# LouisPwr/CarpeDeam

Measured on AMD Instinct MI355X. Metric: corrected bases/sec on 50M×100bp synthetic reads (dhigh), 1/2/4/8 GPU, higher is better.
Workload: dtype u8 (2-bit packed bases; int32 scores; software x87 f80 likelihood sums)

## Files before the change

### carpedeam_amd/csrc/extend.hip

```cpp
#include "scan.h"

#include <cmath>
#include <cstring>

#include "seqdb.h"
#include "devutil.h"

namespace {

struct Cand {
    int qs, qe, ds, de;
    uint32_t target, alnLen, dbLen, qLen;
    float seqId, rySeqId;
    double sLenNorm;
    uint32_t pieceStart, pieceLen;
    uint32_t tKey;
};

struct ExtArgs {
    MetaWoff woff; MetaLen len; MetaHasN hasN; MetaExt ext; MetaKey key; MetaRaw hasRaw;
    const uint32_t *codes, *nmask; const uint8_t *raw;
    const uint64_t *aoff;
    const AlnRec *rec;
    const uint32_t *active; const unsigned int *nActive;
// ... 77 lines not shown
        long long start;
        if (c.ds == 0 && (uint32_t) c.qe == qLen - 1) start = (long long) qLen + c.qs;
        else if (c.qs == 0 && (uint32_t) c.de == tLen - 1) start = (long long) qLen - (long long) (c.dbLen - c.alnLen);
        else continue;
        if ((long long) x < start || (long long) x >= start + (long long) c.dbLen) continue;
        uint32_t tc; bool tn;
        targetBaseAt(A, c.target, (uint32_t) ((long long) x - start), tc, tn);
        cnt[tn ? 0u : fwdBase(tc)]++;
    }
    code = 0; isN = true;
    if (cnt[0] + cnt[1] + cnt[2] + cnt[3] < A.minCov) return;
    uint32_t mx = 0; int nMax = 0;
    for (uint32_t j = 0; j < 4; j++) {
        if (cnt[j] > mx) { mx = cnt[j]; code = j; nMax = 1; } else if (cnt[j] == mx && mx > 0) nMax++;
    }
    isN = nMax != 1;
    if (isN) code = 0;
}


__device__ __forceinline__ bool rightStarts(int ds, int qe, uint32_t qLen) { return (uint32_t) ds == 0 && (uint32_t) qe == (qLen - 1); }
__device__ __forceinline__ bool leftStarts(int qs, int de, uint32_t dbLen) { return (uint32_t) qs == 0 && (uint32_t) de == (dbLen - 1); }

struct Overlap { bool left, right; uint32_t q0, t0, ncol; };
__device__ __forceinline__ Overlap endOverlap(const Cand &c, uint32_t qLen) {
    Overlap o;
    o.right = rightStarts(c.ds, c.qe, qLen); o.left = leftStarts(c.qs, c.de, c.dbLen);
    const uint32_t offset = c.dbLen - c.alnLen;
    if (o.left) { o.t0 = offset; o.q0 = 0; o.ncol = min(c.dbLen - offset, qLen); }
    else { o.t0 = 0; o.q0 = qLen - c.alnLen; o.ncol = min(c.alnLen, c.dbLen); }
    return o;
}
__device__ __forceinline__ void noteOverlap(const Overlap &o, uint32_t tot, uint32_t &maxLeft, uint32_t &maxRight) {
    if (o.left && tot > maxLeft) maxLeft = tot; else if (o.right && tot > maxRight) maxRight = tot;
}
__device__ __forceinline__ void plainOverlapMax(const Cand &c, uint32_t qLen, uint32_t &maxLeft, uint32_t &maxRight) {
    const Overlap o = endOverlap(c, qLen);
    noteOverlap(o, o.ncol, maxLeft, maxRight);
}

__device__ __forceinline__ uint32_t damageClass(uint32_t ti, uint32_t dbLen) { return ti < 5 ? ti : (ti >= dbLen - 5 ? 6 + (ti - (dbLen - 5)) : 5); }

__device__ __forceinline__ void countMatchesWordsAt(const uint32_t *__restrict__ codes, uint32_t qw, uint32_t qLast, uint32_t q0, uint32_t tw, uint32_t tLast, uint32_t t0, uint32_t n, int &idCnt, int &idRy) {
    uint32_t mm = 0, ry = 0;
    for (uint32_t k = 0; k < n; k += 16) {
        const uint32_t x = cdm_window16(codes, qw, q0 + k, qLast) ^ cdm_window16(codes, tw, t0 + k, tLast);
        uint32_t any = (x | (x >> 1)) & 0x55555555u, lowbit = x & 0x55555555u;
        const uint32_t rem = n - k;
        if (rem < 16) { const uint32_t m = (1u << (2 * rem)) - 1u; any &= m; lowbit &= m; }
        mm += __popc(any); ry += __popc(lowbit);
    }
    idCnt = (int) (n - mm); idRy = (int) (n - ry);
}
__device__ __forceinline__ void countMatchesLetters(const ExtArgs &A, uint32_t q, uint32_t qw, uint32_t q0, uint32_t t, uint32_t tw, uint32_t t0, uint32_t n, int &idCnt, int &idRy) {
    idCnt = 0; idRy = 0;
    for (uint32_t i = 0; i < n; i++) {
        uint32_t qc, tc; bool qn, tn;
        letterOf(A, q, qw, q0 + i, qc, qn); letterOf(A, t, tw, t0 + i, tc, tn);
        idCnt += ((qn ? 4u : qc) == (tn ? 4u : tc));
        idRy += (ryClass(qn ? 0u : qc) == ryClass(tn ? 0u : tc));
    }
}

template <typename F>
__device__ __forceinline__ void walkPlainColumns(const ExtArgs &A, const VQuery &Q, const Cand &c, const Overlap &o, F f) {
    const uint32_t qw = Q.qw, tw = A.woff[c.target];
    const uint32_t qLast = (Q.qLen0 + 15) / 16 - 1, tLast = (c.dbLen + 15) / 16 - 1;
    uint32_t qNext = cdm_window16(A.codes, qw, o.q0, qLast), tNext = cdm_window16(A.codes, tw, o.t0, tLast);
    for (uint32_t k = 0; k < o.ncol; k += 16) {
        uint32_t qwin = qNext, twin = tNext;
        if (k + 16 < o.ncol) { qNext = cdm_window16(A.codes, qw, o.q0 + k + 16, qLast); tNext = cdm_window16(A.codes, tw, o.t0 + k + 16, tLast); }
        const uint32_t m = min(16u, o.ncol - k);
        for (uint32_t j = 0; j < m; j++) {
            f(damageClass(o.t0 + k + j, c.dbLen), qwin & 3u, twin & 3u);
            qwin >>= 2; twin >>= 2;
        }
    }
}

__device__ void updateIds(const ExtArgs &A, const VQuery &Q, Cand &c, uint32_t &maxLeft, uint32_t &maxRight, const ConsList *cons = nullptr) {
    const uint32_t qLen = Q.total;
    const Overlap o = endOverlap(c, qLen);
    int idCnt = 0, idRy = 0; uint32_t tot = 0;
    if (cons && (o.left || o.right)) {
        if (c.dbLen - c.alnLen > qLen) A.flags[0] = 1u;
        else {
            const uint32_t c0 = qLen + o.q0 - o.t0;
            for (uint32_t j = 0; j < c.dbLen && c0 + j < 3 * qLen; j++) {
                uint32_t qc, tc; bool qn, tn;
                consensusAt(A, Q, *cons, c0 + j, qc, qn); targetBaseAt(A, c.target, j, tc, tn);
                if (qn || tn) continue;
                idCnt += (qc == tc); idRy += (ryClass(qc) == ryClass(tc)); tot++;
            }
        }
    } else
    if (o.left || o.right) {
        if (Q.plain && !A.hasN[c.target]) {
            countMatchesWordsAt(A.codes, Q.qw, (Q.qLen0 + 15) / 16 - 1, o.q0, A.woff[c.target], (c.dbLen + 15) / 16 - 1, o.t0, o.ncol, idCnt, idRy);
            tot = o.ncol;
        } else
        for (uint32_t i = 0; i < o.ncol; i++) {
            uint32_t qc, tc; bool qn, tn;
            Q.baseAt(o.q0 + i, qc, qn); targetBaseAt(A, c.target, o.t0 + i, tc, tn);
            if (qn || tn) continue;
            idCnt += (qc == tc); idRy += (ryClass(qc) == ryClass(tc)); tot++;
        }
// ... 5 lines not shown
__device__ bool scoreCand(const ExtArgs &A, const VQuery &Q, Cand &c, uint32_t maxLeft, uint32_t maxRight, const double *logLik ,
                          const ConsList *cons = nullptr, const X87 *logLikX = nullptr ) {
    const uint32_t qLen = Q.total;
    const Overlap o = endOverlap(c, qLen);
    const uint32_t maxAln = o.left ? maxLeft : maxRight;
    X87 lik = x87_zero();
    uint32_t alnCount = 0;
    if (cons && (o.left || o.right)) {
        if (c.dbLen - c.alnLen > qLen) A.flags[0] = 1u;
        else {
            const uint32_t c0 = qLen + o.q0 - o.t0;
            uint32_t tIdx = 0;
            for (uint32_t j = 0; j < c.dbLen && c0 + j < 3 * qLen; j++) {
                uint32_t qc, tc; bool qn, tn;
                targetBaseAt(A, c.target, j, tc, tn);
                if (!tn) tIdx++;
                if (tn) continue;
                consensusAt(A, Q, *cons, c0 + j, qc, qn);
                if (qn) continue;
                alnCount++;
                lik = x87_add(lik, x87_from_double(logLik[(damageClass(tIdx - 1, c.dbLen) * 4 + fwdBase(qc)) * 4 + fwdBase(tc)]));
            }
        }
    } else
    if (o.left || o.right) {
        if (Q.plain && !A.hasN[c.target]) {
            if (logLikX) walkPlainColumns(A, Q, c, o, [&](uint32_t cls, uint32_t qb, uint32_t tb) { lik = x87_acc(lik, logLikX[(cls * 4 + qb) * 4 + tb]); });
            else walkPlainColumns(A, Q, c, o, [&](uint32_t cls, uint32_t qb, uint32_t tb) { lik = x87_acc(lik, x87_from_double(logLik[(cls * 4 + qb) * 4 + tb])); });
            alnCount = o.ncol;
        } else {
            uint32_t tIdx = 0;
            if (o.left) for (uint32_t j = 0; j < o.t0; j++) { uint32_t tc; bool tn; targetBaseAt(A, c.target, j, tc, tn); tIdx += !tn; }
            for (uint32_t i = 0; i < o.ncol; i++) {
                uint32_t qc, tc; bool qn, tn;
                Q.baseAt(o.q0 + i, qc, qn); targetBaseAt(A, c.target, o.t0 + i, tc, tn);
                if (!tn) tIdx++;
                if (qn || tn) continue;
                alnCount++;
                lik = x87_add(lik, x87_from_double(logLik[(damageClass(tIdx - 1, c.dbLen) * 4 + fwdBase(qc)) * 4 + fwdBase(tc)]));
            }
        }
    }
    const uint32_t excess = maxAln - alnCount;
    const float pen = (float) excess * A.excessLog;
    lik = x87_add(lik, x87_from_double((double) pen));
    const double randAln = (double) ((float) maxAln * A.randLog);
    c.sLenNorm = x87_to_double(lik);
    X87 neg = lik; neg.s ^= 1u;
    const double x = x87_to_double(x87_add(x87_from_double(randAln), neg));
    if (A.ratioWindow > 0.0 && fabs(x - A.ratioLogit) <= A.ratioWindow) A.flags[2] = 1u;
    return x < A.ratioLogit;
}

__device__ int scoreCandApprox(const ExtArgs &A, const VQuery &Q, const Cand &c, uint32_t maxLeft, uint32_t maxRight, const double *logLik, double &sLenNorm, float &bound) {
    const Overlap o = endOverlap(c, Q.total);
    const uint32_t maxAln = o.left ? maxLeft : maxRight;
    double sum = 0.0, mag = 0.0;
    walkPlainColumns(A, Q, c, o, [&](uint32_t cls, uint32_t qb, uint32_t tb) {
        const double t = logLik[(cls * 4 + qb) * 4 + tb];
        sum = __dadd_rn(sum, t); mag = __dadd_rn(mag, fabs(t));
    });
    const uint32_t excess = maxAln - o.ncol;
    const double pen = (double) ((float) excess * A.excessLog);
    sum = __dadd_rn(sum, pen); mag = __dadd_rn(mag, fabs(pen));
    const double randAln = (double) ((float) maxAln * A.randLog);
    const double b = fmax((double) (o.ncol + 8u) * 0x1p-52 * (mag + fabs(randAln)) * (double) A.marginScale, A.ratioWindow);
    sLenNorm = sum; bound = (float) b * 1.0000002f + 1e-37f;
    const double x = __dadd_rn(randAln, -sum);
    if (x < A.ratioLogit - b) return 1;
    if (x > A.ratioLogit + b) return 0;
    return -1;
}

struct CandTest { bool ok, left, right; uint32_t alnLen; float seqId, rySeqId; };
__device__ __forceinline__ uint32_t recAlnLen(const AlnRec &rec) { return (uint32_t) max(abs(rec.qEnd - rec.qStart), abs(rec.dbEnd - rec.dbStart)) + 1u; }
__device__ __forceinline__ CandTest candidateTest(const ExtArgs &A, const AlnRec &rec, uint32_t q, const SeqMeta &qm, const SeqMeta &tm) {
    CandTest T; T.ok = false; T.alnLen = 0; T.seqId = rec.seqId; T.rySeqId = 0.f;
    T.right = rightStarts(rec.dbStart, rec.qEnd, qm.len); T.left = leftStarts(rec.qStart, rec.dbEnd, tm.len);
    if (!T.right && !T.left) return T;
    if (rec.qStart > rec.qEnd) return T;
    T.alnLen = recAlnLen(rec);
    if (rec.target != qm.key) {
        int idCnt, idRy;
        const uint32_t n = (uint32_t) (rec.qEnd - rec.qStart + 1);
        if (((qm.flags | tm.flags) & 1u) == 0) countMatchesWordsAt(A.codes, qm.woff, (qm.len + 15) / 16 - 1, (uint32_t) rec.qStart, tm.woff, (tm.len + 15) / 16 - 1, (uint32_t) rec.dbStart, n, idCnt, idRy);
        else countMatchesLetters(A, q, qm.woff, (uint32_t) rec.qStart, rec.target, tm.woff, (uint32_t) rec.dbStart, n, idCnt, idRy);
        T.seqId = static_cast<float>(idCnt) / T.alnLen; T.rySeqId = static_cast<float>(idRy) / T.alnLen;
    }
    const bool wasExtended = (tm.flags >> 1) & 1u, noOffset = (tm.len - T.alnLen) == 0;
    T.ok = !wasExtended && T.alnLen >= 30 && T.seqId >= A.seqIdThr && !noOffset;
    return T;
}
__device__ __forceinline__ void candFill(Cand &c, const AlnRec &rec, uint32_t alnLen, const SeqMeta &tm, uint32_t qLen0, float seqId, float rySeqId, uint32_t r) {
    const uint32_t tLen = tm.len; c.tKey = tm.key;
    c.qs = rec.qStart; c.qe = rec.qEnd; c.ds = rec.dbStart; c.de = rec.dbEnd; c.target = rec.target; c.alnLen = alnLen; c.dbLen = tLen;
    c.qLen = qLen0; c.seqId = seqId; c.rySeqId = rySeqId; c.sLenNorm = 0; c.pieceStart = r; c.pieceLen = 0;
}

__device__ __forceinline__ bool scoredAtAll(const ExtArgs &A, const Cand &c, uint32_t qKey) {
    const bool notInside = c.dbLen != c.alnLen, rightStart = c.ds == 0, leftStart = c.qs == 0, notId = c.tKey != qKey;
    return (rightStart || leftStart) && notInside && notId && c.rySeqId >= A.rySeqIdThr && c.seqId >= A.seqIdThr;
}

struct QLists { uint32_t *heap, *park, *left, *right; };
__device__ __forceinline__ QLists queryLists(const ExtArgs &A, uint64_t r0, uint32_t nRec) {
    QLists L; L.heap = A.lists + 4 * r0; L.park = L.heap + nRec; L.left = L.park + nRec; L.right = L.left + nRec;
    return L;
}
__device__ __forceinline__ void queryView(VQuery &Q, const ExtArgs &A, uint32_t q, const SeqMeta &qm, const Cand *cand = nullptr, const QLists *L = nullptr, bool grown = false) {
    Q.a = &A; Q.q = q; Q.qLen0 = qm.len; Q.qw = qm.woff; Q.cand = cand; Q.leftL = L ? L->left : nullptr; Q.rightL = L ? L->right : nullptr;
    Q.nL = grown ? A.nLeft[q] : 0; Q.nR = grown ? A.nRight[q] : 0; Q.leftTotal = grown ? A.leftTotal[q] : 0;
    Q.total = grown ? A.newLen[q] : qm.len; Q.plain = !grown && (qm.flags & 1u) == 0;
}

__device__ __forceinline__ void loadLogLik(const ExtArgs &A, double *sLogLik, X87 *sLogLikX = nullptr) {
    for (int i = threadIdx.x; i < 11 * 16; i += blockDim.x) {
        const double v = (&A.lut->logLik[0][0][0][0])[i];
        sLogLik[i] = v;
        if (sLogLikX) sLogLikX[i] = x87_from_double(v);
    }
}

struct Heap {
    uint32_t *h; uint32_t n; const Cand *cand;
    __device__ bool less(uint32_t x, uint32_t y) const { return cand[x].sLenNorm < cand[y].sLenNorm; }
    __device__ void siftUp(uint32_t hole, uint32_t top, uint32_t value) {
        while (hole > top) { const uint32_t parent = (hole - 1) / 2; if (!less(h[parent], value)) break; h[hole] = h[parent]; hole = parent; }
        h[hole] = value;
    }
    __device__ void push(uint32_t v) { n++; siftUp(n - 1, 0, v); }
    __device__ uint32_t pop() {
        const uint32_t topV = h[0];
        const uint32_t len = n - 1;
        if (len > 0) {
            const uint32_t value = h[len];
            uint32_t hole = 0, child = 0;
            while (child < (len - 1) / 2) { child = 2 * (child + 1); if (less(h[child], h[child - 1])) child--; h[hole] = h[child]; hole = child; }
            if ((len & 1u) == 0 && child == (len - 2) / 2) { child = 2 * (child + 1); h[hole] = h[child - 1]; hole = child - 1; }
// ... 108 lines not shown
    const unsigned int item = blockIdx.x * blockDim.x + threadIdx.x;
    if (item >= *A.nActive) return;
    const uint32_t q = A.active[item];
    const uint64_t r0 = A.aoff[q], r1 = A.aoff[q + 1];
    const uint32_t nRec = (uint32_t) (r1 - r0);
    const SeqMeta *meta = A.len.m;
    const SeqMeta qm = meta[q];
    const uint32_t qLen0 = qm.len, qKey = qm.key;
    Cand *cand = A.cand + r0;
    const QLists L = queryLists(A, r0, nRec);
    VQuery Q; queryView(Q, A, q, qm, cand, &L);

    uint32_t nCand = 0;
    AlnRec recN = A.rec[r0]; SeqMeta tmN = meta[recN.target];
    for (uint32_t r = 0; r < nRec; r++) {
        const AlnRec rec = recN; const SeqMeta tm = tmN;
        if (r + 1 < nRec) { recN = A.rec[r0 + r + 1]; tmN = meta[recN.target]; }
        if (A.scores) A.scores[r0 + r] = NAN;
        const CandTest T = candidateTest(A, rec, q, qm, tm);
        if (T.ok) candFill(cand[nCand++], rec, T.alnLen, tm, qLen0, T.seqId, T.rySeqId, r);
    }
    if (nCand == 0) { A.newLen[q] = 0; return; }
    uint32_t maxLeft = 0, maxRight = 0;
    ConsList consAll; consAll.cand = cand; consAll.idx = nullptr; consAll.n = nCand; consAll.qKey = qKey;
    const ConsList *cons0 = A.unsafe ? &consAll : nullptr;
    for (uint32_t k = 0; k < nCand; k++) {
        Cand &c = cand[k];
        if (A.unsafe) updateIds(A, Q, c, maxLeft, maxRight, cons0);
        else if (Q.plain && !A.hasN[c.target] && c.target != qKey) plainOverlapMax(c, qLen0, maxLeft, maxRight);
        else updateIds(A, Q, c, maxLeft, maxRight);
    }
    Heap heap; heap.h = L.heap; heap.n = 0; heap.cand = cand;
    for (uint32_t k = 0; k < nCand; k++) {
        Cand &c = cand[k];
        if (scoredAtAll(A, c, qKey)) {
            const bool pass = scoreCand(A, Q, c, maxLeft, maxRight, sLogLik, cons0);
            if (A.scores) A.scores[r0 + c.pieceStart] = c.sLenNorm;
            if (pass) heap.push(k);
        }
    }
    extendLoop(A, Q, cand, heap, L, maxLeft, maxRight, sLogLik, qKey, q);
}

constexpr int XR_NT = 512, XR_T = 448, XR_QCAP = 512, XR_LCAP = 1024, XR_BINS = 32;
struct XrArgs {
    const uint32_t *winQ;
    float2 *lite;
    double *sLen;
    float *sBound;
    uint32_t *qMax;
    uint32_t *elig;
    uint32_t *pushBits;
    uint32_t *work; unsigned int *nWork, *fallback;
};
__global__ void k_xr_windows(const uint64_t *__restrict__ aoff, uint32_t n, uint32_t nWin, uint32_t *__restrict__ winQ) {
    const uint32_t b = blockIdx.x * blockDim.x + threadIdx.x;
    if (b > nWin) return;
    const uint64_t x = (uint64_t) b * XR_T;
    uint32_t lo = 0, hi = n;
    while (lo < hi) { const uint32_t mid = lo + (hi - lo) / 2; if (aoff[mid] < x) lo = mid + 1; else hi = mid; }
    winQ[b] = lo;
}
#ifndef CDM_XRS_MINB
#define CDM_XRS_MINB 3
#endif
__global__ __launch_bounds__(XR_NT, CDM_XRS_MINB) void k_xr_score(ExtArgs A, XrArgs X) {
    A.raw = nullptr;
    __shared__ double sLogLik[11 * 16];
    __shared__ X87 sLogLikX[11 * 16];
    __shared__ uint32_t sOff[XR_QCAP + 1], sMaxL[XR_QCAP], sMaxR[XR_QCAP], sCnt[XR_QCAP];
    __shared__ uint32_t sListA[XR_LCAP], sListB[XR_LCAP];
    __shared__ uint8_t sBinOf[XR_LCAP];
    __shared__ unsigned int sElig, sBinCnt[XR_BINS], sBinBase[XR_BINS];
    loadLogLik(A, sLogLik, sLogLikX);
    const uint32_t qFirst = X.winQ[blockIdx.x], qEnd = X.winQ[blockIdx.x + 1];
    const SeqMeta *meta = A.len.m;
    for (uint32_t qb = qFirst; qb < qEnd; qb += XR_QCAP) {
        const uint32_t nq = min((uint32_t) XR_QCAP, qEnd - qb);
        __syncthreads();
        const uint64_t ra = A.aoff[qb];
        for (uint32_t i = threadIdx.x; i <= nq; i += XR_NT) sOff[i] = (uint32_t) (A.aoff[qb + i] - ra);
        for (uint32_t i = threadIdx.x; i < nq; i += XR_NT) { sMaxL[i] = 0; sMaxR[i] = 0; sCnt[i] = 0; }
        if (threadIdx.x == 0) sElig = 0;
        if (threadIdx.x < XR_BINS) sBinCnt[threadIdx.x] = 0;
        __syncthreads();
        const uint32_t nr = sOff[nq];
        for (uint32_t base = 0; base < nr; base += XR_NT) {
            const uint32_t i = base + threadIdx.x;
            if (i >= nr) continue;
            uint32_t lo = 0, hi = nq;
            while (hi - lo > 1) { const uint32_t mid = (lo + hi) / 2; if (sOff[mid] <= i) lo = mid; else hi = mid; }
            const uint32_t ord = lo, q = qb + ord;
            float2 out = make_float2(NAN, 0.f);
            if (sOff[ord + 1] - sOff[ord] > 1) {
                const AlnRec rec = A.rec[ra + i]; const SeqMeta qm = meta[q];
                const bool rightStart = rightStarts(rec.dbStart, rec.qEnd, qm.len);
                const bool maybe = !(rec.qStart > rec.qEnd) && (rightStart || rec.qStart == 0);
                if (maybe) {
                    const SeqMeta tm = meta[rec.target];
                    const CandTest T = candidateTest(A, rec, q, qm, tm);
                    if (T.ok) {
                        Cand c; candFill(c, rec, T.alnLen, tm, qm.len, T.seqId, T.rySeqId, i);
                        if (T.left && T.right) X.fallback[0] = 1u;
                        uint32_t mL = 0, mR = 0;
                        if (((qm.flags | tm.flags) & 1u) == 0 && rec.target != qm.key) plainOverlapMax(c, qm.len, mL, mR);
                        else { VQuery Q; queryView(Q, A, q, qm); updateIds(A, Q, c, mL, mR); }
                        if (mL) atomicMax(&sMaxL[ord], mL);
                        if (mR) atomicMax(&sMaxR[ord], mR);
                        out = make_float2(c.seqId, c.rySeqId);
                        if (scoredAtAll(A, c, qm.key)) {
                            const uint32_t slot = atomicAdd(&sElig, 1u);
                            if (slot < XR_LCAP) {
                                const uint32_t bin = min((uint32_t) XR_BINS - 1u, T.alnLen >> 3);
                                sListA[slot] = i; sBinOf[slot] = (uint8_t) bin; atomicAdd(&sBinCnt[bin], 1u);
                            } else X.elig[ra + slot] = i;
                        }
                    }
                }
            }
            if (out.x == out.x) X.lite[ra + i] = out;
            if (A.scores && sOff[ord + 1] - sOff[ord] > 1) A.scores[ra + i] = NAN;
        }
        __syncthreads();
        const uint32_t nElig = sElig, nListed = min(nElig, (uint32_t) XR_LCAP);
        if (threadIdx.x == 0) { unsigned int acc = 0; for (int b = 0; b < XR_BINS; b++) { sBinBase[b] = acc; acc += sBinCnt[b]; } }
        __syncthreads();
        for (uint32_t k = threadIdx.x; k < nListed; k += XR_NT) sListB[atomicAdd(&sBinBase[sBinOf[k]], 1u)] = sListA[k];
        __syncthreads();
        for (uint32_t k = threadIdx.x; k < nElig; k += XR_NT) {
            const uint32_t i = k < XR_LCAP ? sListB[k] : X.elig[ra + k];
            uint32_t lo = 0, hi = nq;
            while (hi - lo > 1) { const uint32_t mid = (lo + hi) / 2; if (sOff[mid] <= i) lo = mid; else hi = mid; }
            const uint32_t ord = lo, q = qb + ord;
            const float2 l = X.lite[ra + i];
            const AlnRec rec = A.rec[ra + i]; const SeqMeta tm = meta[rec.target], qm = meta[q];
            Cand c; candFill(c, rec, recAlnLen(rec), tm, qm.len, l.x, l.y, i);
            VQuery Q; queryView(Q, A, q, qm);
            bool pass; float bnd = 0.f;
            int quick = -1;
            if (!A.scores && Q.plain && (tm.flags & 1u) == 0) { double sl; quick = scoreCandApprox(A, Q, c, sMaxL[ord], sMaxR[ord], sLogLik, sl, bnd); c.sLenNorm = sl; }
            if (quick < 0) { pass = scoreCand(A, Q, c, sMaxL[ord], sMaxR[ord], sLogLik, nullptr, sLogLikX); bnd = 0.f; }
            else pass = quick != 0;
            if (A.scores) A.scores[ra + i] = c.sLenNorm;
            if (pass) {
                X.sLen[ra + i] = c.sLenNorm; X.sBound[ra + i] = bnd;
                atomicAdd(&sCnt[ord], 1u);
                atomicOr(&X.pushBits[(ra + i) >> 5], 1u << ((ra + i) & 31u));
            }
        }
        __syncthreads();
        for (uint32_t i0 = 0; i0 < nq; i0 += XR_NT) {
            const uint32_t i = i0 + threadIdx.x;
            const bool has = i < nq && sCnt[i] != 0;
            const uint32_t slot = cdm_block_append(X.nWork, has);
            if (has) { X.work[slot] = qb + i; X.qMax[2 * (size_t) (qb + i)] = sMaxL[i]; X.qMax[2 * (size_t) (qb + i) + 1] = sMaxR[i]; }
        }
    }
}

#ifndef CDM_XRE_MINW
#define CDM_XRE_MINW 8
#endif
__global__ __launch_bounds__(64, CDM_XRE_MINW) void k_xr_extend(ExtArgs A, XrArgs X) {
    A.raw = nullptr;
    __shared__ double sLogLik[11 * 16];
    loadLogLik(A, sLogLik);
    __syncthreads();
    const unsigned int item = blockIdx.x * blockDim.x + threadIdx.x;
    if (item >= *X.nWork) return;
    const uint32_t q = X.work[item];
    const SeqMeta *meta = A.len.m;
    const SeqMeta qm = meta[q];
    const uint64_t r0 = A.aoff[q];
    const uint32_t nRec = (uint32_t) (A.aoff[q + 1] - r0);
    Cand *cand = A.cand + r0;
    const QLists L = queryLists(A, r0, nRec);
    VQuery Q; queryView(Q, A, q, qm, cand, &L);
    Heap heap; heap.h = L.heap; heap.n = 0; heap.cand = cand;
    uint32_t nCand = 0;
    const uint32_t maxL0 = X.qMax[2 * (size_t) q], maxR0 = X.qMax[2 * (size_t) q + 1];
    for (uint64_t w = r0 >> 5; w <= (r0 + nRec - 1) >> 5; w++) {
        uint32_t bits = X.pushBits[w];
        if (w == (r0 >> 5)) bits &= ~0u << (r0 & 31u);
        if (w == ((r0 + nRec) >> 5)) bits &= ~(~0u << ((r0 + nRec) & 31u));
        while (bits) {
            const uint32_t b = (uint32_t) __ffs((int) bits) - 1u;
            bits &= bits - 1u;
            const uint64_t ri = (w << 5) + b;
            const AlnRec rec = A.rec[ri]; const float2 l = X.lite[ri];
            Cand c; candFill(c, rec, recAlnLen(rec), meta[rec.target], qm.len, l.x, l.y, (uint32_t) (ri - r0));
            c.sLenNorm = X.sLen[ri];
            c.pieceLen = __float_as_uint(X.sBound[ri]);
            cand[nCand++] = c;
        }
    }
    if (nCand > 1) {
        for (uint32_t i = 0; i < nCand; i++) {
            const float bi = __uint_as_float(cand[i].pieceLen);
            if (!(bi > 0.f)) continue;
            bool open = nCand > 32;
            const double si = cand[i].sLenNorm;
            for (uint32_t j = 0; j < nCand && !open; j++)
                if (j != i) open = fabs(si - cand[j].sLenNorm) <= (double) bi + (double) fabsf(__uint_as_float(cand[j].pieceLen));
            if (open) cand[i].pieceLen |= 0x80000000u;
        }
        for (uint32_t i = 0; i < nCand; i++)
            if (cand[i].pieceLen & 0x80000000u) { Cand c = cand[i]; c.pieceLen = 0; (void) scoreCand(A, Q, c, maxL0, maxR0, sLogLik); cand[i].sLenNorm = c.sLenNorm; }
    }
    for (uint32_t k = 0; k < nCand; k++) { cand[k].pieceLen = 0; heap.push(k); }
// ... 16 lines not shown
        L = newLen[q] ? newLen[q] : len[q];
        oLen[q] = L; oExt[q] = newLen[q] ? 1 : ext[q]; oWords[q] = (L + 15) / 16;
    }
    unsigned long long sum = L; uint32_t mx = L;
    for (int o = 32; o > 0; o >>= 1) { sum += __shfl_xor(sum, o, 64); mx = max(mx, (uint32_t) __shfl_xor((int) mx, o, 64)); }
    __shared__ unsigned long long sSum[16]; __shared__ uint32_t sMax[16];
    if ((threadIdx.x & 63) == 0) { sSum[threadIdx.x >> 6] = sum; sMax[threadIdx.x >> 6] = mx; }
    __syncthreads();
    if (threadIdx.x == 0) {
        for (unsigned w = 1; w < (blockDim.x + 63) / 64; w++) { sum += sSum[w]; mx = max(mx, sMax[w]); }
        atomicAdd(&stats[0], sum); atomicMax(&stats[1], (unsigned long long) mx);
    }
}
__global__ __launch_bounds__(256) void k_write(ExtArgs A, const uint32_t *__restrict__ oWoff, const uint32_t *__restrict__ oLen, uint32_t n,
                                               uint32_t *__restrict__ oCodes, uint32_t *__restrict__ oNmask, uint8_t *__restrict__ oHasN) {
    const uint32_t q = blockIdx.x * blockDim.x + threadIdx.x;
    if (q >= n) return;
    const uint32_t L = oLen[q], nw = (L + 15) / 16, ob = oWoff[q];
    uint16_t *oN16 = reinterpret_cast<uint16_t *>(oNmask);
    uint32_t anyN = 0;
    if (A.newLen[q] == 0) {
        const uint32_t ib = A.woff[q];
        const uint16_t *iN16 = reinterpret_cast<const uint16_t *>(A.nmask);
        for (uint32_t w = 0; w < nw; w++) { const uint32_t nb = iN16[ib + w]; oCodes[ob + w] = A.codes[ib + w]; oN16[ob + w] = (uint16_t) nb; anyN |= nb; }
    } else {
        const uint64_t r0 = A.aoff[q];
        const QLists Ls = queryLists(A, r0, (uint32_t) (A.aoff[q + 1] - r0));
        VQuery Q; queryView(Q, A, q, A.len.m[q], A.cand + r0, &Ls, true);
        for (uint32_t w = 0; w < nw; w++) {
            const uint32_t cnt = min(16u, L - w * 16u);
            uint32_t code = 0, nb = 0;
            for (uint32_t j = 0; j < cnt;) {
                uint32_t t, tp, run;
                Q.spanAt(w * 16 + j, t, tp, run);
                const uint32_t m = min(run, cnt - j), tw = A.woff[t];
                if (!A.hasN[t]) {
                    const uint32_t bits = cdm_window16(A.codes, tw, tp, (A.len[t] + 15) / 16 - 1);
                    code |= ((m < 16) ? (bits & ((1u << (2 * m)) - 1u)) : bits) << (2 * j);
                } else {
                    for (uint32_t i = 0; i < m; i++) {
                        uint32_t c = cdm_base(A.codes, tw, tp + i);
                        if (cdm_isN(A.nmask, tw, tp + i)) { nb |= 1u << (j + i); c = 0; }
                        code |= c << (2 * (j + i));
                    }
                }
                j += m;
            }
            oCodes[ob + w] = code; oN16[ob + w] = (uint16_t) nb; anyN |= nb;
        }
    }
    if (anyN) oHasN[q] = 1;
}

__global__ __launch_bounds__(256) void k_write_raw(ExtArgs A, const uint32_t *__restrict__ oWoff, const uint32_t *__restrict__ oLen, uint32_t n,
                                                   uint8_t *__restrict__ oRaw, uint8_t *__restrict__ oHasN) {
    const uint32_t q = blockIdx.x * blockDim.x + threadIdx.x;
    if (q >= n) return;
    const uint32_t L = oLen[q];
    uint8_t *o = oRaw + (uint64_t) oWoff[q] * 16u;
    const uint64_t r0 = A.aoff[q];
    const QLists Ls = queryLists(A, r0, (uint32_t) (A.aoff[q + 1] - r0));
    VQuery Q; queryView(Q, A, q, A.len.m[q], A.cand + r0, &Ls, A.newLen[q] != 0);
    bool any = false;
    for (uint32_t p = 0; p < L;) { uint32_t t, tp, run; Q.spanAt(p, t, tp, run); any = any || A.hasRaw[t]; p += run; }
    if (!any) return;
    for (uint32_t p = 0; p < L;) {
        uint32_t t, tp, run;
        Q.spanAt(p, t, tp, run);
        const uint32_t tw = A.woff[t], m = min(run, L - p);
        if (A.hasRaw[t]) for (uint32_t i = 0; i < m; i++) o[p + i] = cdm_raw_at(A.raw, tw, tp + i);
        else for (uint32_t i = 0; i < m; i++) o[p + i] = (A.hasN[t] && cdm_isN(A.nmask, tw, tp + i)) ? 'N' : (uint8_t) "ACGT"[cdm_base(A.codes, tw, tp + i)];
        p += m;
    }
    oHasN[q] = 3;
}

}

int cdm_extend_impl(cdm_ctx *ctx, const cdm_seqdb *db, const cdm_alns *alns, const cdm_ancient_params *par, cdm_seqdb **out, double *scores) {
    hipStream_t s = ctx->stream;
    const uint32_t n = (uint32_t) db->n;
    if (alns->n != db->n) { cdm_set_error("cdm_extend: alignment CSR / DB size mismatch"); return CDM_ERR_INVALID; }
    DevBuf<uint32_t> active, lists, newLen, nLeft, nRight, leftTotal, oWords;
    DevBuf<unsigned int> nActive, flags; DevBuf<Cand> cand; DevBuf<double> dScores; DevBuf<unsigned long long> stats;
    if (!active.alloc(n) || !lists.alloc(4 * alns->count) || !newLen.alloc(n) || !nLeft.alloc(n) || !nRight.alloc(n) || !leftTotal.alloc(n) ||
        !oWords.alloc(n) || !nActive.alloc(2) || !flags.alloc(4) || !cand.alloc(alns->count) || !stats.alloc(2) || (scores && !dScores.alloc(alns->count))) {
        cdm_set_error("cdm_extend: out of device memory"); return CDM_ERR_HIP;
    }
    hipMemsetAsync(nActive.p, 0, 8, s);
    hipMemsetAsync(flags.p, 0, 16, s);
    hipMemsetAsync(stats.p, 0, 16, s);
    if (scores) hipMemsetAsync(dScores.p, 0xFF, alns->count * 8, s);
    hipLaunchKernelGGL(k_mark_active2, dim3((n + 1023) / 1024), dim3(1024), 0, s, alns->off, n, active.p, nActive.p, newLen.p);
    unsigned int hAct = 0;
    hipMemcpyAsync(&hAct, nActive.p, 4, hipMemcpyDeviceToHost, s);
    if (hipStreamSynchronize(s) != hipSuccess) { cdm_set_error("cdm_extend: setup failed"); return CDM_ERR_HIP; }
    DevBuf<SeqMeta> meta;
    MetaUniform uni;
    if (int rc = cdm_build_meta(ctx, db, &meta.p, &uni)) return rc;
    ExtArgs A;
    cdmSetMeta(A, meta.p, uni); A.ext.m = A.key.m = meta.p; A.ext.plain = uni.words; A.codes = db->codes; A.nmask = db->nmask; A.raw = db->raw;
    A.aoff = alns->off; A.rec = alns->rec; A.active = active.p; A.nActive = nActive.p; A.lut = ctx->lutDev; A.cand = cand.p; A.lists = lists.p;
    A.newLen = newLen.p; A.nLeft = nLeft.p; A.nRight = nRight.p; A.leftTotal = leftTotal.p; A.scores = scores ? dScores.p : nullptr;
    A.seqIdThr = par->seq_id_thr; A.rySeqIdThr = par->ry_seq_id_thr; A.likelihoodThr = par->likelihood_threshold;
    A.excessLog = std::log(par->excess_penal); A.randLog = std::log(par->rand_align_penal);
    A.ratioLogit = (double) logl(1.0L / (long double) par->likelihood_threshold - 1.0L);
    {
        const double thr = (double) par->likelihood_threshold;
        A.ratioWindow = (par->likelihood_threshold == 0.5f || !(thr > 0.0 && thr < 1.0)) ? 0.0 : 64.0 * 0x1p-53 * (1.0 + fabs(A.ratioLogit) + 1.0 / std::min(thr, 1.0 - thr));
    }
    A.marginScale = cdmGetenv("CDM_EXTEND_MARGIN") ? (float) atof(cdmGetenv("CDM_EXTEND_MARGIN")) : 1.0f;
    A.maxSeqLen = par->max_seq_len;
    A.unsafe = par->unsafe ? 1 : 0; A.minCov = (uint32_t) std::max(0, par->min_cov_safe); A.flags = flags.p;
    hipEventRecord(ctx->ev0, s);
    const char *formEnv = cdmGetenv("CDM_EXTEND");
    bool perRecord = hAct && !db->raw && !A.unsafe && alns->count < 0xFFFFFFFFull / 2 && !(formEnv && !strcmp(formEnv, "queries"));
    DevBuf<uint32_t> winQ, qMax, work, elig, pushBits; DevBuf<float2> lite; DevBuf<double> sLen; DevBuf<float> sBound;
    if (perRecord) {
        const uint32_t nWin = (uint32_t) ((alns->count + XR_T - 1) / XR_T);
        if (!winQ.alloc((size_t) nWin + 1) || !qMax.alloc(2 * (size_t) n) || !work.alloc(hAct) || !lite.alloc(alns->count) || !sLen.alloc(alns->count) ||
            !elig.alloc(alns->count) || !pushBits.alloc(alns->count / 32 + 2) || !sBound.alloc(alns->count)) {
            cdm_set_error("cdm_extend: out of device memory"); return CDM_ERR_HIP;
        }
        hipMemsetAsync(pushBits.p, 0, (alns->count / 32 + 2) * 4, s);
        XrArgs X; X.sBound = sBound.p; X.elig = elig.p; X.pushBits = pushBits.p; X.winQ = winQ.p; X.lite = lite.p; X.sLen = sLen.p; X.qMax = qMax.p; X.work = work.p; X.nWork = nActive.p + 1; X.fallback = flags.p + 1;
        hipLaunchKernelGGL(k_xr_windows, dim3(nWin / 256 + 1), dim3(256), 0, s, alns->off, n, nWin, winQ.p);
        hipLaunchKernelGGL(k_xr_score, CDM_GRID(nWin, XR_NT), dim3(XR_NT), 0, s, A, X);
        unsigned int fb = 0;
        hipMemcpyAsync(&fb, flags.p + 1, 4, hipMemcpyDeviceToHost, s);
        if (hipStreamSynchronize(s) != hipSuccess) { cdm_set_error("cdm_extend: scoring kernel failed"); return CDM_ERR_HIP; }
        if (fb) perRecord = false;
        else hipLaunchKernelGGL(k_xr_extend, dim3((hAct + 63) / 64), dim3(64), 0, s, A, X);
    }
    if (perRecord) {}
    else if (hAct && db->raw) hipLaunchKernelGGL((k_extend<8, true>), dim3((hAct + 63) / 64), dim3(64), 0, s, A);
    else if (hAct) hipLaunchKernelGGL((k_extend<8, false>), dim3((hAct + 63) / 64), dim3(64), 0, s, A);
    hipEventRecord(ctx->ev1, s);
    cdm_seqdb *o = nullptr;
    int rc = cdm_seqdb_alloc(ctx, n, &o);
    if (rc) return rc;
    hipLaunchKernelGGL(k_out_meta, dim3((n + 1023) / 1024), dim3(1024), 0, s, db->len, db->ext, newLen.p, n, o->len, o->ext, oWords.p, stats.p);
    cdmscan::ScanTemp tmp;
    hipMemsetAsync(oWords.p + n, 0, 4, s);
    if (cdmscan::exclusiveScan<uint32_t>(s, tmp, oWords.p, o->woff, (size_t) n + 1) != CDM_OK) { cdm_seqdb_free(o); return CDM_ERR_HIP; }
    uint32_t words = 0; unsigned long long hstats[2] = {0, 0}; unsigned int hflags[4] = {0, 0, 0, 0};
    hipMemcpyAsync(hflags, flags.p, 16, hipMemcpyDeviceToHost, s);
    hipMemcpyAsync(&words, o->woff + n, 4, hipMemcpyDeviceToHost, s);
    hipMemcpyAsync(hstats, stats.p, 16, hipMemcpyDeviceToHost, s);
    { hipError_t e = hipStreamSynchronize(s); if (e != hipSuccess) { cdm_seqdb_free(o); cdm_set_error("cdm_extend: extension kernel failed: %s", hipGetErrorString(e)); return CDM_ERR_HIP; } }
    hipEventElapsedTime(&ctx->lastMs[4], ctx->ev0, ctx->ev1);
    if (hflags[0]) {
        cdm_seqdb_free(o);
        cdm_set_error("cdm_extend: --unsafe 1: a target overhangs the query by more than the query's length; the reference pads it with a negative number of letters there (undefined behaviour), not reproduced");
        return CDM_ERR_UNSUPPORTED;
    }
    if (hflags[2]) {
        cdm_seqdb_free(o);
        cdm_set_error("cdm_extend: --likelihood-ratio-threshold %g: a candidate's likelihood ratio lies within %.3g of the threshold in log-odds; the reference decides there by the last bit of the C library's expl - not reproduced (the default threshold 0.5 has no such window)", (double) par->likelihood_threshold, A.ratioWindow);
        return CDM_ERR_UNSUPPORTED;
    }
    if (hstats[0] / 16 + n >= 0xFFFFFFF0ull) {
        cdm_seqdb_free(o); cdm_set_error("cdm_extend: the extended sequences need more than 2^32 code words (68 G bases) in one DB"); return CDM_ERR_UNSUPPORTED;
    }
    o->residues = hstats[0]; o->maxLen = (uint32_t) hstats[1];
    if (seqdbAllocPlanes(o, words, false) != CDM_OK) { cdm_seqdb_free(o); cdm_set_error("cdm_extend: out of device memory"); return CDM_ERR_HIP; }
    hipMemcpyAsync(o->key, db->key, (size_t) n * 4, hipMemcpyDeviceToDevice, s);
    hipMemsetAsync(o->hasN, 0, n, s);
    if (words) hipLaunchKernelGGL(k_write, dim3((n + 255) / 256), dim3(256), 0, s, A, o->woff, o->len, n, o->codes, o->nmask, o->hasN);
    if (words && db->raw) {
        if (int rc2 = cdm_seqdb_alloc_raw(o)) { cdm_seqdb_free(o); return rc2; }
        hipLaunchKernelGGL(k_write_raw, dim3((n + 255) / 256), dim3(256), 0, s, A, o->woff, o->len, n, o->raw, o->hasN);
    }
    if (scores) hipMemcpyAsync(scores, dScores.p, alns->count * 8, hipMemcpyDeviceToHost, s);
    { hipError_t e = hipStreamSynchronize(s); if (e != hipSuccess) { cdm_seqdb_free(o); cdm_set_error("cdm_extend: output kernel failed: %s", hipGetErrorString(e)); return CDM_ERR_HIP; } }
    *out = o;
    return CDM_OK;
}
```

Baseline: 18.09 billion.

## Count interior matches by base class, chunk word loads, parallelize output write

The approximate scorer now loads packed code words in chunks and handles interior matching columns by popcount per base class, multiplying each count by its log-likelihood instead of adding every column. Only mismatches and damage-zone columns are still summed one by one. The candidate identity count gets the same chunked loads, and a new word-parallel output kernel, with block-level binary search over queries, replaces the per-sequence writer. The scoring kernel's launch attributes change, and an optional stats kernel is added; multiplied sums can round differently than sequential adds, though the error bound still guards the decision.

```diff
diff --git a/carpedeam_amd/csrc/extend.hip b/carpedeam_amd/csrc/extend.hip
--- a/carpedeam_amd/csrc/extend.hip
+++ b/carpedeam_amd/csrc/extend.hip
@@ -153,6 +153,34 @@
     }
     idCnt = (int) (n - mm); idRy = (int) (n - ry);
 }
+#ifndef CDM_XR_CHUNK
+#define CDM_XR_CHUNK 4
+#endif
+constexpr uint32_t XC = CDM_XR_CHUNK;
+__device__ __forceinline__ void countMatchesWordsChunked(const uint32_t *__restrict__ codes, uint32_t qw, uint32_t qLast, uint32_t q0, uint32_t tw, uint32_t tLast, uint32_t t0, uint32_t n, int &idCnt, int &idRy) {
+    uint32_t mm = 0, ry = 0;
+    for (uint32_t kc = 0; kc < n; kc += 16 * XC) {
+        const uint32_t qp = q0 + kc, tp = t0 + kc, qs = (qp & 15u) * 2u, ts = (tp & 15u) * 2u;
+        uint32_t qv[XC + 1], tv[XC + 1];
+#pragma unroll
+        for (uint32_t j = 0; j <= XC; j++) {
+            const uint32_t a = (qp >> 4) + j, b = (tp >> 4) + j;
+            qv[j] = (a <= qLast && 16 * j <= n - kc + 15u) ? codes[qw + a] : 0u;
+            tv[j] = (b <= tLast && 16 * j <= n - kc + 15u) ? codes[tw + b] : 0u;
+        }
+#pragma unroll
+        for (uint32_t j = 0; j < XC; j++) {
+            const uint32_t k = kc + 16 * j;
+            if (k >= n) break;
+            const uint32_t x = (qs ? ((qv[j] >> qs) | (qv[j + 1] << (32u - qs))) : qv[j]) ^ (ts ? ((tv[j] >> ts) | (tv[j + 1] << (32u - ts))) : tv[j]);
+            uint32_t any = (x | (x >> 1)) & 0x55555555u, lowbit = x & 0x55555555u;
+            const uint32_t rem = n - k;
+            if (rem < 16) { const uint32_t m = (1u << (2 * rem)) - 1u; any &= m; lowbit &= m; }
+            mm += __popc(any); ry += __popc(lowbit);
+        }
+    }
+    idCnt = (int) (n - mm); idRy = (int) (n - ry);
+}
 __device__ __forceinline__ void countMatchesLetters(const ExtArgs &A, uint32_t q, uint32_t qw, uint32_t q0, uint32_t t, uint32_t tw, uint32_t t0, uint32_t n, int &idCnt, int &idRy) {
     idCnt = 0; idRy = 0;
     for (uint32_t i = 0; i < n; i++) {
@@ -264,14 +292,60 @@
     return x < A.ratioLogit;
 }
 
+__device__ __forceinline__ uint32_t evenBitsBelow(uint32_t n) { return n >= 16u ? 0x55555555u : (((1u << (2u * n)) - 1u) & 0x55555555u); }
+
+template <bool COUNTS>
 __device__ int scoreCandApprox(const ExtArgs &A, const VQuery &Q, const Cand &c, uint32_t maxLeft, uint32_t maxRight, const double *logLik, double &sLenNorm, float &bound) {
     const Overlap o = endOverlap(c, Q.total);
     const uint32_t maxAln = o.left ? maxLeft : maxRight;
     double sum = 0.0, mag = 0.0;
-    walkPlainColumns(A, Q, c, o, [&](uint32_t cls, uint32_t qb, uint32_t tb) {
-        const double t = logLik[(cls * 4 + qb) * 4 + tb];
-        sum = __dadd_rn(sum, t); mag = __dadd_rn(mag, fabs(t));
-    });
+    if (!COUNTS) {
+        walkPlainColumns(A, Q, c, o, [&](uint32_t cls, uint32_t qb, uint32_t tb) {
+            const double t = logLik[(cls * 4 + qb) * 4 + tb];
+            sum = __dadd_rn(sum, t); mag = __dadd_rn(mag, fabs(t));
+        });
+    } else {
+        const uint32_t qw = Q.qw, tw = A.woff[c.target];
+        const uint32_t qLast = (Q.qLen0 + 15) / 16 - 1, tLast = (c.dbLen + 15) / 16 - 1;
+        for (uint32_t k0 = 0; k0 < o.ncol; k0 += 32768u) {
+            uint64_t nb = 0;
+            const uint32_t kEnd = min(o.ncol, k0 + 32768u);
+            for (uint32_t kc = k0; kc < kEnd; kc += 16 * XC) {
+                const uint32_t qp = o.q0 + kc, tp = o.t0 + kc, qs = (qp & 15u) * 2u, ts = (tp & 15u) * 2u;
+                uint32_t qv[XC + 1], tv[XC + 1];
+#pragma unroll
+                for (uint32_t j = 0; j <= XC; j++) {
+                    const uint32_t a = (qp >> 4) + j, b = (tp >> 4) + j;
+                    qv[j] = (a <= qLast && 16 * j <= kEnd - kc + 15u) ? A.codes[qw + a] : 0u;
+                    tv[j] = (b <= tLast && 16 * j <= kEnd - kc + 15u) ? A.codes[tw + b] : 0u;
+                }
+#pragma unroll
+                for (uint32_t j = 0; j < XC; j++) {
+                    const uint32_t k = kc + 16 * j;
+                    if (k >= kEnd) break;
+                    const uint32_t qwin = qs ? ((qv[j] >> qs) | (qv[j + 1] << (32u - qs))) : qv[j], twin = ts ? ((tv[j] >> ts) | (tv[j + 1] << (32u - ts))) : tv[j];
+                    const uint32_t ti = o.t0 + k;
+                    const uint32_t valid = evenBitsBelow(o.ncol - k);
+                    const uint32_t inLo = ti < 5u ? 5u - ti : 0u, inHi = c.dbLen - 5u > ti ? c.dbLen - 5u - ti : 0u;
+                    const uint32_t interior = inHi > inLo ? (evenBitsBelow(inHi) & ~evenBitsBelow(inLo)) : 0u;
+                    const uint32_t x = qwin ^ twin;
+                    const uint32_t counted = valid & interior & ~(x | (x >> 1));
+                    const uint32_t l = qwin, h = qwin >> 1;
+                    nb += (uint64_t) (__popc(counted & ~l & ~h) | (__popc(counted & l & ~h) << 16)) | ((uint64_t) (__popc(counted & ~l & h) | (__popc(counted & l & h) << 16)) << 32);
+                    for (uint32_t rest = valid & ~counted; rest; rest &= rest - 1u) {
+                        const uint32_t sh = (uint32_t) __ffs((int) rest) - 1u;
+                        const double t = logLik[(damageClass(ti + (sh >> 1), c.dbLen) * 4 + ((qwin >> sh) & 3u)) * 4 + ((twin >> sh) & 3u)];
+                        sum = __dadd_rn(sum, t); mag = __dadd_rn(mag, fabs(t));
+                    }
+                }
+            }
+#pragma unroll
+            for (uint32_t b = 0; b < 4; b++) {
+                const double t = __dmul_rn((double) (uint32_t) ((nb >> (16 * b)) & 0xFFFFu), logLik[(5 * 4 + b) * 4 + b]);
+                sum = __dadd_rn(sum, t); mag = __dadd_rn(mag, fabs(t));
+            }
+        }
+    }
     const uint32_t excess = maxAln - o.ncol;
     const double pen = (double) ((float) excess * A.excessLog);
     sum = __dadd_rn(sum, pen); mag = __dadd_rn(mag, fabs(pen));
@@ -286,6 +360,7 @@
 
 struct CandTest { bool ok, left, right; uint32_t alnLen; float seqId, rySeqId; };
 __device__ __forceinline__ uint32_t recAlnLen(const AlnRec &rec) { return (uint32_t) max(abs(rec.qEnd - rec.qStart), abs(rec.dbEnd - rec.dbStart)) + 1u; }
+template <bool CHUNKED = false>
 __device__ __forceinline__ CandTest candidateTest(const ExtArgs &A, const AlnRec &rec, uint32_t q, const SeqMeta &qm, const SeqMeta &tm) {
     CandTest T; T.ok = false; T.alnLen = 0; T.seqId = rec.seqId; T.rySeqId = 0.f;
     T.right = rightStarts(rec.dbStart, rec.qEnd, qm.len); T.left = leftStarts(rec.qStart, rec.dbEnd, tm.len);
@@ -295,7 +370,10 @@
     if (rec.target != qm.key) {
         int idCnt, idRy;
         const uint32_t n = (uint32_t) (rec.qEnd - rec.qStart + 1);
-        if (((qm.flags | tm.flags) & 1u) == 0) countMatchesWordsAt(A.codes, qm.woff, (qm.len + 15) / 16 - 1, (uint32_t) rec.qStart, tm.woff, (tm.len + 15) / 16 - 1, (uint32_t) rec.dbStart, n, idCnt, idRy);
+        if (((qm.flags | tm.flags) & 1u) == 0) {
+            if (CHUNKED) countMatchesWordsChunked(A.codes, qm.woff, (qm.len + 15) / 16 - 1, (uint32_t) rec.qStart, tm.woff, (tm.len + 15) / 16 - 1, (uint32_t) rec.dbStart, n, idCnt, idRy);
+            else countMatchesWordsAt(A.codes, qm.woff, (qm.len + 15) / 16 - 1, (uint32_t) rec.qStart, tm.woff, (tm.len + 15) / 16 - 1, (uint32_t) rec.dbStart, n, idCnt, idRy);
+        }
         else countMatchesLetters(A, q, qm.woff, (uint32_t) rec.qStart, rec.target, tm.woff, (uint32_t) rec.dbStart, n, idCnt, idRy);
         T.seqId = static_cast<float>(idCnt) / T.alnLen; T.rySeqId = static_cast<float>(idRy) / T.alnLen;
     }
@@ -510,6 +588,7 @@
     uint32_t *elig;
     uint32_t *pushBits;
     uint32_t *work; unsigned int *nWork, *fallback;
+    unsigned long long *stats;
 };
 __global__ void k_xr_windows(const uint64_t *__restrict__ aoff, uint32_t n, uint32_t nWin, uint32_t *__restrict__ winQ) {
     const uint32_t b = blockIdx.x * blockDim.x + threadIdx.x;
@@ -522,7 +601,8 @@
 #ifndef CDM_XRS_MINB
 #define CDM_XRS_MINB 3
 #endif
-__global__ __launch_bounds__(XR_NT, CDM_XRS_MINB) void k_xr_score(ExtArgs A, XrArgs X) {
+template <bool COUNTS>
+__global__ __attribute__((amdgpu_flat_work_group_size(XR_NT, XR_NT), amdgpu_waves_per_eu(CDM_XRS_MINB * (XR_NT / 64) / 4, 8))) void k_xr_score(ExtArgs A, XrArgs X) {
     A.raw = nullptr;
     __shared__ double sLogLik[11 * 16];
     __shared__ X87 sLogLikX[11 * 16];
@@ -556,7 +636,7 @@
                 const bool maybe = !(rec.qStart > rec.qEnd) && (rightStart || rec.qStart == 0);
                 if (maybe) {
                     const SeqMeta tm = meta[rec.target];
-                    const CandTest T = candidateTest(A, rec, q, qm, tm);
+                    const CandTest T = candidateTest<COUNTS>(A, rec, q, qm, tm);
                     if (T.ok) {
                         Cand c; candFill(c, rec, T.alnLen, tm, qm.len, T.seqId, T.rySeqId, i);
                         if (T.left && T.right) X.fallback[0] = 1u;
@@ -596,7 +676,7 @@
             VQuery Q; queryView(Q, A, q, qm);
             bool pass; float bnd = 0.f;
             int quick = -1;
-            if (!A.scores && Q.plain && (tm.flags & 1u) == 0) { double sl; quick = scoreCandApprox(A, Q, c, sMaxL[ord], sMaxR[ord], sLogLik, sl, bnd); c.sLenNorm = sl; }
+            if (!A.scores && Q.plain && (tm.flags & 1u) == 0) { double sl; quick = scoreCandApprox<COUNTS>(A, Q, c, sMaxL[ord], sMaxR[ord], sLogLik, sl, bnd); c.sLenNorm = sl; }
             if (quick < 0) { pass = scoreCand(A, Q, c, sMaxL[ord], sMaxR[ord], sLogLik, nullptr, sLogLikX); bnd = 0.f; }
             else pass = quick != 0;
             if (A.scores) A.scores[ra + i] = c.sLenNorm;
@@ -613,6 +693,21 @@
             const uint32_t slot = cdm_block_append(X.nWork, has);
             if (has) { X.work[slot] = qb + i; X.qMax[2 * (size_t) (qb + i)] = sMaxL[i]; X.qMax[2 * (size_t) (qb + i) + 1] = sMaxR[i]; }
         }
+        if (X.stats && threadIdx.x == 0) atomicAdd(&X.stats[0], (unsigned long long) nElig);
+    }
+}
+
+__global__ void k_xr_stats(XrArgs X, const uint64_t *__restrict__ aoff, uint64_t count) {
+    const uint64_t stride = (uint64_t) gridDim.x * blockDim.x, t0 = (uint64_t) blockIdx.x * blockDim.x + threadIdx.x;
+    unsigned int nCand = 0;
+    for (uint64_t r = t0; r < count; r += stride) { const float v = X.lite[r].x; nCand += v == v; }
+    if (nCand) atomicAdd(&X.stats[1], (unsigned long long) nCand);
+    for (uint64_t k = t0; k < *X.nWork; k += stride) {
+        const uint32_t q = X.work[k];
+        unsigned int c = 0;
+        for (uint64_t r = aoff[q]; r < aoff[q + 1]; r++) c += (X.pushBits[r >> 5] >> (r & 31u)) & 1u;
+        const int bin = c <= 1 ? 0 : min(6, 32 - __clz((int) (c - 1u)));
+        atomicAdd(&X.stats[2], (unsigned long long) c); atomicAdd(&X.stats[3 + bin], 1ull);
     }
 }
 
@@ -735,6 +830,81 @@
     if (anyN) oHasN[q] = 1;
 }
 
+constexpr int XW_Q = 256, XW_U = 7;
+__global__ __launch_bounds__(XW_Q) void k_write_words(ExtArgs A, const uint32_t *__restrict__ oWoff, const uint32_t *__restrict__ oLen, uint32_t n,
+                                                      uint32_t *__restrict__ oCodes, uint32_t *__restrict__ oNmask, uint8_t *__restrict__ oHasN) {
+    __shared__ uint32_t sW[XW_Q + 1], sNew[XW_Q], sIn[XW_Q], sAnyN[XW_Q], sX[XW_Q];
+    const uint32_t q0 = blockIdx.x * XW_Q, nq = min((uint32_t) XW_Q, n - q0);
+    for (uint32_t i = threadIdx.x; i <= XW_Q; i += XW_Q) sW[i] = i <= nq ? oWoff[q0 + i] : 0xFFFFFFFFu;
+    sNew[threadIdx.x] = threadIdx.x < nq ? A.newLen[q0 + threadIdx.x] : 0u;
+    sIn[threadIdx.x] = threadIdx.x < nq ? A.woff[q0 + threadIdx.x] : 0u;
+    sAnyN[threadIdx.x] = 0;
+    __syncthreads();
+    const uint32_t w0 = sW[0], w1 = sW[nq];
+    uint16_t *oN16 = reinterpret_cast<uint16_t *>(oNmask);
+    const uint16_t *iN16 = reinterpret_cast<const uint16_t *>(A.nmask);
+    for (uint32_t base = w0 + threadIdx.x; base < w1; base += XW_Q * XW_U) {
+        uint32_t own[XW_U], code[XW_U], nb[XW_U];
+#pragma unroll
+        for (int u = 0; u < XW_U; u++) own[u] = 0;
+#pragma unroll
+        for (uint32_t step = XW_Q / 2; step > 0; step >>= 1) {
+#pragma unroll
+            for (int u = 0; u < XW_U; u++) own[u] += sW[own[u] + step] <= base + u * XW_Q ? step : 0u;
+        }
+#pragma unroll
+        for (int u = 0; u < XW_U; u++) {
+            const uint32_t ow = base + u * XW_Q, lo = own[u];
+            const bool copy = ow < w1 && sNew[lo] == 0;
+            const uint32_t src = copy ? sIn[lo] + (ow - sW[lo]) : 0u;
+            if (!copy) own[u] = 0xFFFFFFFFu;
+            code[u] = A.codes[src]; nb[u] = iN16[src];
+        }
+#pragma unroll
+        for (int u = 0; u < XW_U; u++) {
+            if (own[u] == 0xFFFFFFFFu) continue;
+            const uint32_t ow = base + u * XW_Q;
+            oCodes[ow] = code[u]; oN16[ow] = (uint16_t) nb[u];
+            if (nb[u]) atomicOr(&sAnyN[own[u]], 1u);
+        }
+    }
+    uint32_t nx = 0;
+    const uint32_t mine = (threadIdx.x < nq && sNew[threadIdx.x]) ? sW[threadIdx.x + 1] - sW[threadIdx.x] : 0u;
+    sX[threadIdx.x] = cdm_block_excl_sum<uint32_t>(mine, nx);
+    __syncthreads();
+    for (uint32_t x = threadIdx.x; x < nx; x += XW_Q) {
+        uint32_t lo = 0;
+#pragma unroll
+        for (uint32_t step = XW_Q / 2; step > 0; step >>= 1) lo += sX[lo + step] <= x ? step : 0u;
+        const uint32_t q = q0 + lo, w = x - sX[lo];
+        const uint64_t r0 = A.aoff[q];
+        const QLists Ls = queryLists(A, r0, (uint32_t) (A.aoff[q + 1] - r0));
+        VQuery Q; queryView(Q, A, q, A.len.m[q], A.cand + r0, &Ls, true);
+        const uint32_t cnt = min(16u, oLen[q] - w * 16u);
+        uint32_t code = 0, nb = 0;
+        for (uint32_t j = 0; j < cnt;) {
+            uint32_t t, tp, run;
+            Q.spanAt(w * 16 + j, t, tp, run);
+            const uint32_t m = min(run, cnt - j), tw = A.woff[t];
+            if (!A.hasN[t]) {
+                const uint32_t bits = cdm_window16(A.codes, tw, tp, (A.len[t] + 15) / 16 - 1);
+                code |= ((m < 16) ? (bits & ((1u << (2 * m)) - 1u)) : bits) << (2 * j);
+            } else {
+                for (uint32_t i = 0; i < m; i++) {
+                    uint32_t c = cdm_base(A.codes, tw, tp + i);
+                    if (cdm_isN(A.nmask, tw, tp + i)) { nb |= 1u << (j + i); c = 0; }
+                    code |= c << (2 * (j + i));
+                }
+            }
+            j += m;
+        }
+        oCodes[sW[lo] + w] = code; oN16[sW[lo] + w] = (uint16_t) nb;
+        if (nb) atomicOr(&sAnyN[lo], 1u);
+    }
+    __syncthreads();
+    if (threadIdx.x < nq && sAnyN[threadIdx.x]) oHasN[q0 + threadIdx.x] = 1;
+}
+
 __global__ __launch_bounds__(256) void k_write_raw(ExtArgs A, const uint32_t *__restrict__ oWoff, const uint32_t *__restrict__ oLen, uint32_t n,
                                                    uint8_t *__restrict__ oRaw, uint8_t *__restrict__ oHasN) {
     const uint32_t q = blockIdx.x * blockDim.x + threadIdx.x;
@@ -806,12 +976,25 @@
             cdm_set_error("cdm_extend: out of device memory"); return CDM_ERR_HIP;
         }
         hipMemsetAsync(pushBits.p, 0, (alns->count / 32 + 2) * 4, s);
-        XrArgs X; X.sBound = sBound.p; X.elig = elig.p; X.pushBits = pushBits.p; X.winQ = winQ.p; X.lite = lite.p; X.sLen = sLen.p; X.qMax = qMax.p; X.work = work.p; X.nWork = nActive.p + 1; X.fallback = flags.p + 1;
+        DevBuf<unsigned long long> xrStats;
+        const bool wantStats = cdmGetenv("CDM_XR_STATS") && xrStats.alloc(10);
+        if (wantStats) { hipMemsetAsync(xrStats.p, 0, 80, s); hipMemsetAsync(lite.p, 0xFF, alns->count * sizeof(float2), s); }
+        XrArgs X; X.stats = wantStats ? xrStats.p : nullptr; X.sBound = sBound.p; X.elig = elig.p; X.pushBits = pushBits.p; X.winQ = winQ.p; X.lite = lite.p; X.sLen = sLen.p; X.qMax = qMax.p; X.work = work.p; X.nWork = nActive.p + 1; X.fallback = flags.p + 1;
         hipLaunchKernelGGL(k_xr_windows, dim3(nWin / 256 + 1), dim3(256), 0, s, alns->off, n, nWin, winQ.p);
-        hipLaunchKernelGGL(k_xr_score, CDM_GRID(nWin, XR_NT), dim3(XR_NT), 0, s, A, X);
+        const char *sumEnv = cdmGetenv("CDM_XR_SUM");
+        if (sumEnv && !strcmp(sumEnv, "columns")) hipLaunchKernelGGL(k_xr_score<false>, CDM_GRID(nWin, XR_NT), dim3(XR_NT), 0, s, A, X);
+        else hipLaunchKernelGGL(k_xr_score<true>, CDM_GRID(nWin, XR_NT), dim3(XR_NT), 0, s, A, X);
         unsigned int fb = 0;
         hipMemcpyAsync(&fb, flags.p + 1, 4, hipMemcpyDeviceToHost, s);
         if (hipStreamSynchronize(s) != hipSuccess) { cdm_set_error("cdm_extend: scoring kernel failed"); return CDM_ERR_HIP; }
+        if (wantStats && !fb) {
+            unsigned long long st[10]; unsigned int nw = 0;
+            hipLaunchKernelGGL(k_xr_stats, dim3(ctx->cuCount * 8), dim3(256), 0, s, X, alns->off, (uint64_t) alns->count);
+            hipMemcpyAsync(st, xrStats.p, 80, hipMemcpyDeviceToHost, s); hipMemcpyAsync(&nw, nActive.p + 1, 4, hipMemcpyDeviceToHost, s);
+            if (hipStreamSynchronize(s) == hipSuccess)
+                fprintf(stderr, "xr: %u queries on the work list of %u with records; pushed records per query 1: %llu, 2: %llu, 3-4: %llu, 5-8: %llu, 9-16: %llu, 17-32: %llu, >32: %llu; "
+                        "records: %llu, candidates %llu, scored %llu, pushed %llu\n", nw, hAct, st[3], st[4], st[5], st[6], st[7], st[8], st[9], (unsigned long long) alns->count, st[1], st[0], st[2]);
+        }
         if (fb) perRecord = false;
         else hipLaunchKernelGGL(k_xr_extend, dim3((hAct + 63) / 64), dim3(64), 0, s, A, X);
     }
@@ -849,7 +1032,9 @@
     if (seqdbAllocPlanes(o, words, false) != CDM_OK) { cdm_seqdb_free(o); cdm_set_error("cdm_extend: out of device memory"); return CDM_ERR_HIP; }
     hipMemcpyAsync(o->key, db->key, (size_t) n * 4, hipMemcpyDeviceToDevice, s);
     hipMemsetAsync(o->hasN, 0, n, s);
-    if (words) hipLaunchKernelGGL(k_write, dim3((n + 255) / 256), dim3(256), 0, s, A, o->woff, o->len, n, o->codes, o->nmask, o->hasN);
+    const char *writeEnv = cdmGetenv("CDM_EXTEND_WRITE");
+    if (words && writeEnv && !strcmp(writeEnv, "seq")) hipLaunchKernelGGL(k_write, dim3((n + 255) / 256), dim3(256), 0, s, A, o->woff, o->len, n, o->codes, o->nmask, o->hasN);
+    else if (words) hipLaunchKernelGGL(k_write_words, dim3((n + XW_Q - 1) / XW_Q), dim3(XW_Q), 0, s, A, o->woff, o->len, n, o->codes, o->nmask, o->hasN);
     if (words && db->raw) {
         if (int rc2 = cdm_seqdb_alloc_raw(o)) { cdm_seqdb_free(o); return rc2; }
         hipLaunchKernelGGL(k_write_raw, dim3((n + 255) / 256), dim3(256), 0, s, A, o->woff, o->len, n, o->raw, o->hasN);
```

New measurement: 18.25 billion (median of 6 runs). About the same (+0.9%).
